# yflyzhang/RankPO

Hardware: AMD Instinct MI355X
Metric: query-passage pairs/sec (higher is better)
Workload: dtype bf16

## Files before the change

include/rankpo_hip.h:

```cpp
#ifndef RANKPO_HIP_H
#define RANKPO_HIP_H

#include <stddef.h>
#include <stdint.h>

#ifdef __cplusplus
extern "C" {
#endif

typedef void* rpo_stream_t;

typedef enum {
    RPO_OK = 0,
    RPO_ERR_INVALID_ARG = -1,
    RPO_ERR_UNSUPPORTED = -2,
    RPO_ERR_WORKSPACE = -3,
    RPO_ERR_LAUNCH = -4
} rpo_status;

typedef enum { RPO_DT_F32 = 0, RPO_DT_BF16 = 1, RPO_DT_F16 = 2 } rpo_dtype;
typedef enum { RPO_POOL_LAST = 0, RPO_POOL_CLS = 1 } rpo_pool_mode;
typedef enum { RPO_TARGET_INBATCH = 0, RPO_TARGET_FIRST = 1 } rpo_target_mode;
typedef enum { RPO_LOSS_SIGMOID = 0, RPO_LOSS_HINGE = 1 } rpo_loss_type;

// ... 86 lines not shown
                          int dtype, float lr, float beta1, float beta2, float eps, float weight_decay, const void* ls_state,
                          rpo_stream_t stream);

int rpo_swiglu_fwd(const void* g, const void* u, void* out, int64_t rows, int64_t cols, int64_t ld_gu, int64_t ld_out,
                   int dtype, rpo_stream_t stream);
int rpo_swiglu_bwd(const void* g, const void* u, const void* dout, void* dg, void* du, void* prod_out, int64_t rows,
                   int64_t cols, int64_t ld_gu, int64_t ld_dout, int64_t ld_dgu, int64_t ld_prod, int dtype,
                   rpo_stream_t stream);
int rpo_swiglu_bwd_t(const void* g, const void* u, const void* dout, void* dg, void* du, void* prod_t_out, void* dgu_t_out,
                     int64_t rows, int64_t cols, int64_t ld_gu, int64_t ld_dout, int64_t ld_dgu, int64_t ld_t, int dtype,
                     rpo_stream_t stream);
int rpo_rope(const void* x_in, void* x_out, int64_t row_stride, const float* cos_tab, const float* sin_tab,
             int64_t rows, int64_t heads, int64_t head_dim, int64_t period, int dtype, int backward,
             rpo_stream_t stream);

int rpo_transpose(const void* in, void* out, int64_t rows, int64_t cols, int64_t ld_in, int64_t ld_out, int dtype,
                  rpo_stream_t stream);

int rpo_add_rmsnorm_waves(int64_t rows);
int rpo_add_rmsnorm_fwd(const void* x, const void* delta, const void* weight, float eps, void* x_out, void* y_out,
                        float* rstd_out, int64_t rows, int64_t d, int dtype, rpo_stream_t stream);
int rpo_add_rmsnorm_bwd(const void* dy, const void* x_new, const void* weight, const float* rstd, const void* dres,
                        void* dx_out, float* dw_partial, int64_t rows, int64_t d, int dtype, rpo_stream_t stream);

int rpo_flash_attn_fwd(const void* q, const void* k, const void* v, int64_t q_stride, int64_t k_stride,
                       int64_t v_stride, const int* cu_seqlens, const int* tiles, int64_t ntiles, int64_t tile_cols,
                       int64_t total_tokens,
                       int64_t num_heads, int64_t num_kv_heads, int64_t head_dim, float scale, void* out,
                       int64_t out_stride, float* lse, int64_t lse_max_len, const float* rope_cos, const float* rope_sin,
                       int64_t rope_period, int64_t q_block, rpo_stream_t stream);

int rpo_flash_attn_bwd(const void* q, const void* k, const void* v, const void* out, const void* dout, int64_t q_stride,
                       int64_t k_stride, int64_t v_stride, int64_t out_stride, int64_t dout_stride,
                       const int* cu_seqlens, const int* q_tiles, int64_t n_q_tiles, int64_t q_tile_cols, const int* k_tiles,
                       int64_t n_k_tiles, int64_t key_block, int64_t sweep_down, int64_t total_tokens, int64_t num_heads,
                       int64_t num_kv_heads, int64_t head_dim, float scale, const float* lse, float* delta, void* dq, void* dk, void* dv,
                       int64_t dq_stride, int64_t dk_stride, int64_t dv_stride, const float* rope_cos, const float* rope_sin,
                       int64_t rope_period, int64_t q_block, rpo_stream_t stream);

int rpo_lastq_attn_fwd(const void* q, int64_t q_stride, const void* k, const void* v, int64_t k_stride, int64_t v_stride,
                       const int* cu_seqlens, int64_t num_seqs, int64_t num_heads, int64_t num_kv_heads, int64_t head_dim,
                       float scale, void* out, int64_t out_stride, float* lse, rpo_stream_t stream);
int rpo_lastq_attn_bwd(const void* q, int64_t q_stride, const void* k, const void* v, int64_t k_stride, int64_t v_stride,
                       const int* cu_seqlens, int64_t num_seqs, int64_t num_heads, int64_t num_kv_heads, int64_t head_dim,
                       float scale, const void* out, int64_t out_stride, const void* dout, int64_t dout_stride, const float* lse,
                       void* dq, int64_t dq_stride, void* dk, void* dv, int64_t dk_stride, int64_t dv_stride, rpo_stream_t stream);
// ... 65 lines not shown
                 int dtype, rpo_stream_t stream);

float rpo_hidden_dropout_scale(float p_drop);
int rpo_add_layernorm_drop_fwd(const void* a, int64_t lda, const void* b, int64_t ldb, const void* gamma, const void* beta,
                               float eps, void* y, int64_t ldy, void* s, int64_t lds, int64_t rows, int64_t d, int dtype,
                               float p_drop, uint64_t seed, int64_t site, rpo_stream_t stream);
int rpo_bert_embed_ln_drop_fwd(const int* ids, const int* token_types, const int* pos, int64_t tokens, const void* word,
                               int64_t vocab, const void* type_emb, int64_t n_types, const void* pos_emb, int64_t n_pos,
                               const void* gamma, const void* beta, float eps, void* y, int64_t ldy, void* s, int64_t lds,
                               int64_t d, int dtype, float p_drop, uint64_t seed, int64_t site, rpo_stream_t stream);
int rpo_layernorm_drop_bwd(const void* s, int64_t lds, const void* gamma, const void* dy, int64_t lddy, float eps, void* ds,
                           int64_t ldds, void* db, int64_t lddb, float* dgamma_partial, float* dbeta_partial, int64_t rows,
                           int64_t d, int dtype, float p_drop, uint64_t seed, int64_t site_in, int64_t site_out,
                           rpo_stream_t stream);
int rpo_hidden_dropout_mask(int64_t row0, int64_t rows, int64_t d, float p_drop, uint64_t seed, int64_t site,
                            unsigned char* mask, rpo_stream_t stream);

int64_t rpo_embed_grad_workspace_elems(int64_t n_partials, int64_t d);
int rpo_embed_grad_sorted(const void* ds, int64_t ldds, int64_t tokens, int64_t d, int dtype, const int* order, const int* chunks,
                          int64_t n_chunks, const int* multi, int64_t n_multi, int64_t n_partials, void* out, int64_t ldout,
                          int64_t table_rows, int64_t padding_idx, float* workspace, int64_t workspace_elems,
                          rpo_stream_t stream);

int rpo_topk_merge(const void* scores, int64_t ld, int64_t rows, int64_t cols, int64_t col0, int k, int dtype,
                   float* best_val, int64_t* best_idx, int first, rpo_stream_t stream);
int rpo_topk_merge_split(const void* scores, int64_t ld, int64_t rows, int64_t cols, int64_t col0, int k, int dtype, int split,
                         float* best_val, int64_t* best_idx, int first, rpo_stream_t stream);

int rpo_sim_topk_filter_ok(int64_t Q, int64_t P, int64_t d);
int rpo_sim_topk_filter(const void* q, const void* p, int64_t Q, int64_t P, int64_t d, int dtype, int64_t col0, int k,
                        int round_scores, const float* best_val, const int64_t* best_idx, float* cand_val, int64_t* cand_idx,
                        int32_t* cand_cnt, int cap, rpo_stream_t stream);
int rpo_sim_scores_f32(const void* q, const void* p, int64_t Q, int64_t P, int64_t d, int dtype, float* scores, int64_t ldc,
                       rpo_stream_t stream);
int rpo_topk_merge_candidates(const float* cand_val, const int64_t* cand_idx, int32_t* cand_cnt, int64_t rows, int cap, int k,
                              float* best_val, int64_t* best_idx, int32_t* overflow, rpo_stream_t stream);

int rpo_split_bf16x3(const float* x, int64_t ldx, int64_t rows, int64_t d, void* planes, int64_t ldp, int32_t* inexact,
                     rpo_stream_t stream);
int rpo_sim_planes_ok(int64_t Q, int64_t P, int64_t d);
int rpo_sim_scores_f32_planes(const void* q, const void* p, int64_t Q, int64_t P, int64_t d, float* scores, int64_t ldc,
                              rpo_stream_t stream);
int rpo_sim_topk_filter_planes(const void* q, const void* p, int64_t Q, int64_t P, int64_t d, int64_t col0, int k,
                               const float* best_val, const int64_t* best_idx, float* cand_val, int64_t* cand_idx,
                               int32_t* cand_cnt, int cap, rpo_stream_t stream);

// ... 5 lines not shown
```

rankpo_amd/_lib.py:

```python
from __future__ import annotations

import ctypes as C
import os

_HERE = os.path.dirname(os.path.abspath(__file__))
LIB_PATH = os.path.join(_HERE, "csrc", "librankpo_hip.so")

RPO_OK = 0
RPO_DT_F32, RPO_DT_BF16, RPO_DT_F16 = 0, 1, 2
RPO_POOL_LAST, RPO_POOL_CLS = 0, 1
(RPO_LS_SCALE, RPO_LS_MULT, RPO_LS_NORM, RPO_LS_SKIP, RPO_LS_GOOD_STEPS, RPO_LS_CUR_HYSTERESIS, RPO_LS_APPLIED_STEPS,
 RPO_LS_SKIPPED_STEPS, RPO_LS_FLOOR_HITS) = range(9)
RPO_LS_WORDS = 16
RPO_TARGET_INBATCH, RPO_TARGET_FIRST = 0, 1
RPO_LOSS_SIGMOID, RPO_LOSS_HINGE = 0, 1
RPO_BUILD_ONEWAVE64 = 1
RPO_NUM_METRICS = 9
METRIC_KEYS = (
    "rankpo_loss", "sft_loss", "rewards/chosen", "rewards/rejected", "rewards/accuracies",
    "rewards/margins", "scores/chosen", "scores/rejected", "scores/margins",
)


class RankPOParams(C.Structure):
# ... 75 lines not shown
                                           _i32, _f32, _f32, _u64, _vp, _i64, _vp, _vp]),
    "rpo_bidir_attn_bwd": (C.c_int, [_vp, _vp, _vp, _i64, _i64, _i64, _vp, _i64, _vp, _i64, _vp, _vp, _vp, _vp, _i64, _vp, _i64,
                                     _i64, _i64, _i64, _i64, _i64, _i64, _i32, _f32, _f32, _u64, _vp, _i64, _vp, _i64, _vp, _i64,
                                     _vp]),
    "rpo_bidir_attn_dropout_mask": (C.c_int, [_i64, _i64, _i64, _i64, _i64, _i64, _f32, _u64, _vp, _vp]),
    "rpo_add_layernorm_train_fwd": (C.c_int, [_vp, _i64, _vp, _i64, _vp, _vp, _f32, _vp, _i64, _vp, _i64, _i64, _i64, _i32, _vp]),
    "rpo_bert_embed_ln_train_fwd": (C.c_int, [_vp, _vp, _vp, _i64, _vp, _i64, _vp, _i64, _vp, _i64, _vp, _vp, _f32, _vp, _i64, _vp,
                                              _i64, _i64, _i32, _vp]),
    "rpo_layernorm_bwd_blocks": (C.c_int, [_i64]),
    "rpo_layernorm_bwd": (C.c_int, [_vp, _i64, _vp, _vp, _i64, _f32, _vp, _i64, _vp, _vp, _i64, _i64, _i32, _vp]),
    "rpo_gelu_out_fwd": (C.c_int, [_vp, _i64, _vp, _i64, _i64, _i64, _i32, _vp]),
    "rpo_gelu_bwd": (C.c_int, [_vp, _i64, _vp, _i64, _vp, _i64, _i64, _i64, _i32, _vp]),
    "rpo_hidden_dropout_scale": (_f32, [_f32]),
    "rpo_add_layernorm_drop_fwd": (C.c_int, [_vp, _i64, _vp, _i64, _vp, _vp, _f32, _vp, _i64, _vp, _i64, _i64, _i64, _i32, _f32, _u64,
                                             _i64, _vp]),
    "rpo_bert_embed_ln_drop_fwd": (C.c_int, [_vp, _vp, _vp, _i64, _vp, _i64, _vp, _i64, _vp, _i64, _vp, _vp, _f32, _vp, _i64, _vp,
                                             _i64, _i64, _i32, _f32, _u64, _i64, _vp]),
    "rpo_layernorm_drop_bwd": (C.c_int, [_vp, _i64, _vp, _vp, _i64, _f32, _vp, _i64, _vp, _i64, _vp, _vp, _i64, _i64, _i32, _f32,
                                         _u64, _i64, _i64, _vp]),
    "rpo_hidden_dropout_mask": (C.c_int, [_i64, _i64, _i64, _f32, _u64, _i64, _vp, _vp]),
    "rpo_embed_grad_workspace_elems": (_i64, [_i64, _i64]),
    "rpo_embed_grad_sorted": (C.c_int, [_vp, _i64, _i64, _i64, _i32, _vp, _vp, _i64, _vp, _i64, _i64, _vp, _i64, _i64, _i64, _vp,
                                        _i64, _vp]),
}

_lib = None


def load():
    global _lib
    if _lib is not None:
        return _lib
    if not os.path.exists(LIB_PATH):
        raise ImportError(
            f"{LIB_PATH} not found: the HIP scoring library is not built.  Run "
            "`python -c 'import __graft_entry__ as g; g.build()'` (or `make -C rankpo_amd/csrc`).  "
            "rankpo_amd has no CPU fallback for its hot path.")
    import torch
    lib = C.CDLL(LIB_PATH)
    for name, (res, args) in SIGNATURES.items():
        try:
            fn = getattr(lib, name)
        except AttributeError as e:
            raise ImportError(f"{LIB_PATH} does not export {name}; rebuild it (make -C rankpo_amd/csrc)") from e
        fn.restype = res
        fn.argtypes = args
# ... 11 lines not shown
```

rankpo_amd/csrc/embed_grad.hip:

```cpp
#include "common.hpp"

namespace {

constexpr int kEgWaves = 4;
constexpr int kEgSliceCols = 512;

template <typename T> __device__ __forceinline__ void add_row(float (&acc)[8], const Vec16<T>& x) {
#pragma unroll
    for (int j = 0; j < 8; ++j) acc[j] += x.v[j];
}

template <typename T> __device__ __forceinline__ void store_rounded(T* p, const float (&acc)[8]) {
    Vec16<T> r;
#pragma unroll
    for (int j = 0; j < 8; ++j) r.v[j] = acc[j];
    r.store(p);
}

template <typename T>
__global__ __launch_bounds__(64 * kEgWaves) void embed_grad_chunk_kernel(
    const T* __restrict__ ds, int64_t ldds, int tokens, int d, const int* __restrict__ order, const int* __restrict__ chunks,
    int64_t n_chunks, int64_t n_partials, T* __restrict__ out, int64_t ldout, int64_t table_rows, int64_t padding_idx,
    float* __restrict__ ws) {
    const int wave = __builtin_amdgcn_readfirstlane((int)(threadIdx.x >> 6));
// ... 45 lines not shown
    const int* __restrict__ multi, int64_t n_multi, int d, int64_t n_partials, const float* __restrict__ ws,
    T* __restrict__ out, int64_t ldout, int64_t table_rows, int64_t padding_idx) {
    const int wave = __builtin_amdgcn_readfirstlane((int)(threadIdx.x >> 6));
    const int64_t m = (int64_t)blockIdx.x * kEgWaves + wave;
    if (m >= n_multi) return;
    const int slice = (int)blockIdx.y;
    const int* mu = multi + 3 * m;
    const int row = mu[0], slot0 = mu[1], k = mu[2];
    if (row < 0 || row >= table_rows || row == padding_idx || slot0 < 0 || k < 1 || (int64_t)slot0 + k > n_partials) return;
    const int col = slice * kEgSliceCols + (int)(threadIdx.x & 63) * 8;
    if (col >= d) return;
    const float* p = ws + (int64_t)slot0 * d + col;
    float acc[8];
#pragma unroll
    for (int j = 0; j < 8; ++j) acc[j] = 0.f;
    for (int i = 0; i < k; ++i, p += d) {
        const float4 a = *reinterpret_cast<const float4*>(p), b = *reinterpret_cast<const float4*>(p + 4);
        acc[0] += a.x; acc[1] += a.y; acc[2] += a.z; acc[3] += a.w;
        acc[4] += b.x; acc[5] += b.y; acc[6] += b.z; acc[7] += b.w;
    }
    store_rounded<T>(out + (int64_t)row * ldout + col, acc);
}

}

extern "C" int64_t rpo_embed_grad_workspace_elems(int64_t n_partials, int64_t d) {
    return n_partials <= 0 || d <= 0 ? 0 : n_partials * d;
}

extern "C" int rpo_embed_grad_sorted(const void* ds, int64_t ldds, int64_t tokens, int64_t d, int dtype, const int* order,
                                     const int* chunks, int64_t n_chunks, const int* multi, int64_t n_multi, int64_t n_partials,
                                     void* out, int64_t ldout, int64_t table_rows, int64_t padding_idx, float* workspace,
                                     int64_t workspace_elems, rpo_stream_t stream) {
    if (!ds || !out || tokens < 0 || tokens > INT32_MAX || d <= 0 || table_rows <= 0 || table_rows > INT32_MAX || ldds < d ||
        ldout < d || !rpo_dtype_ok(dtype) || n_chunks < 0 || n_multi < 0 || n_partials < 0 || padding_idx < -1 ||
        padding_idx >= table_rows || (n_chunks > 0 && (!order || !chunks)) || (n_multi > 0 && !multi) ||
        (n_partials > 0 && !workspace) || (n_multi > 0) != (n_partials > 0))
        return RPO_ERR_INVALID_ARG;
    if (dtype == RPO_DT_F32 || d % 8 || d > 65535 * (int64_t)kEgSliceCols) return RPO_ERR_UNSUPPORTED;
    if (!rpo_aligned16(ds) || !rpo_aligned16(out) || ldds % 8 || ldout % 8 || (n_partials > 0 && !rpo_aligned16(workspace)))
        return RPO_ERR_UNSUPPORTED;
    if (workspace_elems < rpo_embed_grad_workspace_elems(n_partials, d)) return RPO_ERR_WORKSPACE;
    if (tokens == 0 || n_chunks == 0) return RPO_OK;
    const unsigned nslices = (unsigned)rpo_cdiv(d, kEgSliceCols);
    if (n_chunks > INT32_MAX || n_multi > INT32_MAX) return RPO_ERR_UNSUPPORTED;
    const dim3 block(64 * kEgWaves), grid1((unsigned)rpo_cdiv(n_chunks, kEgWaves), nslices),
// ... 19 lines not shown
```

rankpo_amd/csrc/encoder_ops.hip:

```cpp
#include "common.hpp"

namespace {

constexpr int kEwThreads = 256;

__device__ __forceinline__ float sigmoid_f(float x) { return 1.0f / (1.0f + __expf(-x)); }

template <typename T>
__global__ __launch_bounds__(kEwThreads) void swiglu_fwd_kernel(const T* __restrict__ g, const T* __restrict__ u,
                                                                T* __restrict__ out, int64_t rows, int vec_per_row,
                                                                int64_t ld_gu, int64_t ld_out) {
    constexpr int V = Elem<T>::kVec;
    const int64_t i = (int64_t)blockIdx.x * kEwThreads + threadIdx.x;
    const int64_t r = i / vec_per_row;
    if (r >= rows) return;
    const int c = (int)(i - r * vec_per_row) * V;
    Vec16<T> a, b, o;
    a.load_nt(g + r * ld_gu + c);
    b.load_nt(u + r * ld_gu + c);
#pragma unroll
    for (int k = 0; k < V; ++k) o.v[k] = a.v[k] * sigmoid_f(a.v[k]) * b.v[k];
    o.store_nt(out + r * ld_out + c);
}

// ... 551 lines not shown
        (delta && (!rpo_aligned16(delta) || !rpo_aligned16(x_out))))
        return RPO_ERR_UNSUPPORTED;
    hipStream_t st = (hipStream_t)stream;
    const int nw = norm_waves(rows, RPO_NORM_FWD_CAP);
    if (dtype == RPO_DT_BF16) return launch_norm_fwd<bf16_t>(x, delta, weight, eps, x_out, y_out, rstd_out, rows, d, nw, st);
    if (dtype == RPO_DT_F32) return launch_norm_fwd<float>(x, delta, weight, eps, x_out, y_out, rstd_out, rows, d, nw, st);
    return RPO_ERR_INVALID_ARG;
}

extern "C" int rpo_add_rmsnorm_bwd(const void* dy, const void* x_new, const void* weight, const float* rstd,
                                   const void* dres, void* dx_out, float* dw_partial, int64_t rows, int64_t d,
                                   int dtype, rpo_stream_t stream) {
    if (!dy || !x_new || !weight || !rstd || !dx_out || !dw_partial || rows <= 0 || d <= 0) return RPO_ERR_INVALID_ARG;
    const int V = dtype == RPO_DT_BF16 ? 8 : 4;
    if (d % V != 0 || !rpo_aligned16(dy) || !rpo_aligned16(x_new) || !rpo_aligned16(dx_out) || !rpo_aligned16(weight) ||
        !rpo_aligned16(dw_partial) || (dres && !rpo_aligned16(dres)))
        return RPO_ERR_UNSUPPORTED;
    hipStream_t st = (hipStream_t)stream;
    const int nw = rpo_add_rmsnorm_waves(rows);
    if (dtype == RPO_DT_BF16) return launch_norm_bwd<bf16_t>(dy, x_new, weight, rstd, dres, dx_out, dw_partial, rows, d, nw, st);
    if (dtype == RPO_DT_F32) return launch_norm_bwd<float>(dy, x_new, weight, rstd, dres, dx_out, dw_partial, rows, d, nw, st);
    return RPO_ERR_INVALID_ARG;
}
```

rankpo_amd/encoder.py:

```python
from __future__ import annotations

import functools
import json
import math
import os
from types import SimpleNamespace
from typing import Optional

import torch
import torch.nn.functional as F
from torch import nn
from torch.utils.checkpoint import checkpoint

from . import ops as _ops


class EncoderConfig(SimpleNamespace):

    def to_dict(self):
        return dict(self.__dict__)

    @classmethod
    def from_json_file(cls, path):
        with open(path) as f:
# ... 507 lines not shown
            o += n + 2
        if not all(oks):
            return None
        ids_parts, pos_parts = [], []
        for ids, m in batches:
            L = m.shape[1]
            flat = torch.nonzero(m.reshape(-1).to(torch.bool), as_tuple=False).squeeze(1)
            ids_parts.append(ids.reshape(-1)[flat])
            pos_parts.append(flat % L)
        n_fill = 0
        if (dev.type == "cuda" and self.embed_tokens.weight.dtype == torch.bfloat16 and sum(lens) >= 4096
                and self.pack_fill):
            n_fill = (-sum(lens)) % 256
        if n_fill:
            pad_id = self.config.pad_token_id if self.config.pad_token_id is not None else 0
            ids_parts.append(torch.full((n_fill,), pad_id, dtype=ids_parts[0].dtype, device=ids_parts[0].device))
            pos_parts.append(torch.arange(n_fill, dtype=pos_parts[0].dtype, device=pos_parts[0].device))
            lens = lens + [n_fill]
        ids = ids_parts[0] if len(ids_parts) == 1 else torch.cat(ids_parts)
        pos = pos_parts[0] if len(pos_parts) == 1 else torch.cat(pos_parts)
        if on_host:
            both = torch.stack([ids.to(torch.int32), pos.to(torch.int32)]).pin_memory().to(dev, non_blocking=True)
            ids, pos = both[0], both[1]
        x = self.embed_tokens(ids)[None]
        rope = self._rope(pos)
        N = len(lens)
        cu = torch.zeros(N + 1, dtype=torch.int32, device=x.device)
        cu[1:] = torch.tensor(lens, dtype=torch.int64).cumsum(0).to(torch.int32).to(x.device, non_blocking=True)
        tiles = k_tiles = fwd_tiles = None
        if (x.is_cuda and self.config.head_dim in (64, 128) and x.dtype == torch.bfloat16
                and self.hand_attention):
            tiles = _ops.attn_tile_table(lens, x.device, self.config.num_attention_heads, self.config.num_key_value_heads)
            if FWD128_ONE_WAVE:
                fwd_tiles = _ops.attn_fwd_tile_table(lens, x.device, self.config.num_attention_heads,
                                                     self.config.num_key_value_heads, self.config.head_dim)
            if torch.is_grad_enabled():
                k_tiles = _ops.attn_key_tile_table(
                    lens, x.device, self.config.num_key_value_heads,
                    _ops.ATTN_KEY_BLOCK if self.config.head_dim == 64 else _ops.ATTN_KEY_BLOCK_HD128)
        f32_tiles = f32_last_tiles = None
        if ((LLAMA_F32_ATTENTION or self.f32_attention) and x.is_cuda and x.dtype == torch.float32 and not torch.is_grad_enabled()
                and _ops.causal_attn_f32_shape_ok(self.config.num_attention_heads, self.config.num_key_value_heads,
                                                  self.config.head_dim)):
            f32_tiles = _ops.causal_attn_f32_tile_table(lens, lens, x.device)
            f32_last_tiles = _ops.causal_attn_f32_tile_table([1] * N, lens, x.device)
        f32_k_tiles = f32_last_k_tiles = None
        if ((LLAMA_F32_ATTENTION_TRAIN or self.f32_attention_train) and x.is_cuda and x.dtype == torch.float32
# ... 553 lines not shown
```

rankpo_amd/ops.py:

```python
from __future__ import annotations

import ctypes as C
import threading
from dataclasses import dataclass
from typing import NamedTuple

import torch

from . import _lib
from ._lib import (RPO_DT_BF16, RPO_DT_F16, RPO_DT_F32, RPO_LOSS_HINGE, RPO_LOSS_SIGMOID, RPO_NUM_METRICS, RPO_POOL_CLS,
                   RPO_POOL_LAST, RPO_TARGET_FIRST, RPO_TARGET_INBATCH, METRIC_KEYS, RankPOParams, check)

F_NORMALIZE_EPS = 1e-12


def _dt(t: torch.Tensor) -> int:
    if t.dtype == torch.float32:
        return RPO_DT_F32
    if t.dtype == torch.bfloat16:
        return RPO_DT_BF16
    if t.dtype == torch.float16:
        return RPO_DT_F16
    raise TypeError(f"rankpo_amd HIP kernels take float32, bfloat16 or float16 tensors, got {t.dtype}")


# ... 240 lines not shown


def rankpo_loss_metrics(q, p, cfg: RankPOConfig, ref_chosen=None, ref_rejected=None):
    return _RankPO.apply(q, p, ref_chosen, ref_rejected, cfg)


def _swiglu_fwd(lib, gu, prod, rows, ff):
    es = gu.element_size()
    with torch.cuda.device(gu.device):
        check(lib.rpo_swiglu_fwd(gu.data_ptr(), gu.data_ptr() + ff * es, prod.data_ptr(), rows, ff, 2 * ff, ff, _dt(gu),
                                 _stream(gu)), "rpo_swiglu_fwd")
    return prod


LINEAR_TN = True
WGRAD_MIXED = True
SWIGLU_DGU_T = True
SWIGLU_DGU_T_DEFAULT_MAX_BYTES = 6 * 2 ** 30
SWIGLU_DGU_T_MAX_BYTES = SWIGLU_DGU_T_DEFAULT_MAX_BYTES
SWIGLU_PROD_T = True
WGRAD_SPLIT_T = 4


def transpose2d(x):
    _need_gpu(x)
    lib = _lib.load()
    if x.dim() != 2 or x.stride(1) != 1:
        raise ValueError("transpose2d: a 2-D tensor with contiguous rows")
    R, C_ = x.shape
    out = torch.empty((C_, R), dtype=x.dtype, device=x.device)
    with torch.cuda.device(x.device):
        check(lib.rpo_transpose(x.data_ptr(), out.data_ptr(), R, C_, x.stride(0), R, _dt(x), _stream(x)), "rpo_transpose")
    return out


WGRAD_DY_T_HITS = 0


def wgrad(dy2, x2, dy_t=None):
    n, k = dy2.shape[1], x2.shape[1]
    if dy_t is not None and tuple(dy_t.shape) == (n, dy2.shape[0]) and dy_t.dtype == dy2.dtype and x2.stride(1) == 1:
        global WGRAD_DY_T_HITS
        WGRAD_DY_T_HITS += 1
        return torch.nn.functional.linear(dy_t, transpose2d(x2))
    if WGRAD_MIXED and dy2.is_cuda and dy2.dtype == torch.bfloat16 and dy2.stride(1) == 1 and x2.stride(1) == 1:
        if n >= 2 * k:
            return dy2.t() @ transpose2d(x2).t()
        if k >= 2 * n:
            return transpose2d(dy2) @ x2
        T, S = dy2.shape[0], WGRAD_SPLIT_T
        if S > 1 and T >= 32768 and T % S == 0 and n * k <= 8 * 1024 * 1024 and dy2.is_contiguous() and x2.is_contiguous():
            if _bmm_f32_out_ok(dy2.device):
                part = torch.bmm(dy2.view(S, T // S, n).transpose(1, 2), x2.view(S, T // S, k), out_dtype=torch.float32)
                return part.sum(0).to(dy2.dtype)
    return dy2.t() @ x2


_BMM_F32_OUT = {}


def _bmm_f32_out_ok(device) -> bool:
    key = str(device)
    if key not in _BMM_F32_OUT:
        try:
            a = torch.ones(2, 8, 16, dtype=torch.bfloat16, device=device)
            r = torch.bmm(a.transpose(1, 2), a, out_dtype=torch.float32)
            _BMM_F32_OUT[key] = bool(r.dtype == torch.float32 and float(r[0, 0, 0]) == 8.0)
        except Exception:
            _BMM_F32_OUT[key] = False
    return _BMM_F32_OUT[key]


def _wt(w):
    return transpose2d(w) if w.is_cuda and w.dtype in (torch.bfloat16, torch.float16, torch.float32) and w.stride(1) == 1 else w.t().contiguous()


# ... 132 lines not shown
        return x_new, y

    @staticmethod
    def backward(ctx, *grads):
        x_new, weight, rstd = ctx.saved_tensors
        lib = _lib.load()
        if ctx.has_delta:
            dres, dy = grads
        else:
            dres, dy = None, grads[0]
        d = x_new.shape[-1]
        rows = x_new.numel() // d
        if dy is None:
            return dres, (dres if ctx.has_delta else None), None, None
        dy = dy.contiguous()
        dres = None if dres is None else dres.contiguous()
        dx = torch.empty_like(x_new)
        nw = lib.rpo_add_rmsnorm_waves(rows)
        dwp = torch.empty((nw, d), dtype=torch.float32, device=x_new.device)
        with torch.cuda.device(x_new.device):
            check(lib.rpo_add_rmsnorm_bwd(dy.data_ptr(), x_new.data_ptr(), weight.data_ptr(), rstd.data_ptr(), _p(dres),
                                          dx.data_ptr(), dwp.data_ptr(), rows, d, _dt(x_new), _stream(x_new)),
                  "rpo_add_rmsnorm_bwd")
        dw = dwp.sum(0).to(weight.dtype) if ctx.needs_input_grad[2] else None
        return dx, (dx if ctx.has_delta else None), dw, None


def add_rmsnorm(x, delta, weight, eps):
    if delta is None:
        return x, _AddRMSNorm.apply(x, None, weight, eps)
    return _AddRMSNorm.apply(x, delta, weight, eps)


def fused_norm_ok(x) -> bool:
    if not x.is_cuda or x.dtype not in (torch.float32, torch.bfloat16):
        return False
    v = 8 if x.dtype == torch.bfloat16 else 4
    d = x.shape[-1]
    return d % v == 0 and d // v <= 64 * 8


class _Rope(torch.autograd.Function):

    @staticmethod
    def forward(ctx, x, cos, sin, heads, head_dim, grad_inplace):
        lib = _lib.load()
        row_len = x.shape[-1]
# ... 876 lines not shown
    return _AddLayerNorm.apply(a, b, weight, bias, eps, p_drop, seed, site)


def embed_grad_sorted(ds, plan: EmbedGradPlan, table_rows: int, padding_idx=None):
    lib = _lib.load()
    T, d = ds.shape
    if plan.order.shape[0] != T:
        raise ValueError("embed_grad_sorted: the plan was built for another number of tokens")
    ds = ds if ds.stride(1) == 1 and ds.stride(0) % 8 == 0 and ds.data_ptr() % 16 == 0 else ds.contiguous()
    out = torch.zeros((table_rows, d), dtype=ds.dtype, device=ds.device)
    if T == 0:
        return out
    ws_elems = lib.rpo_embed_grad_workspace_elems(plan.n_partials, d)
    ws = torch.empty((ws_elems,), dtype=torch.float32, device=ds.device) if ws_elems else None
    with torch.cuda.device(ds.device):
        check(lib.rpo_embed_grad_sorted(ds.data_ptr(), ds.stride(0), T, d, _dt(ds), plan.order.data_ptr(), plan.chunks.data_ptr(),
                                        plan.chunks.shape[0], plan.multi.data_ptr() if plan.multi.shape[0] else None,
                                        plan.multi.shape[0], plan.n_partials, out.data_ptr(), d, table_rows,
                                        -1 if padding_idx is None else int(padding_idx), _p(ws), ws_elems, _stream(ds)),
              "rpo_embed_grad_sorted")
    return out


class _BertEmbedLayerNorm(torch.autograd.Function):

    @staticmethod
    def forward(ctx, ids, pos, token_types, word, type_emb, pos_emb, weight, bias, eps, padding_idx, p_drop=0.0, seed=0,
                plans=None):
        lib = _lib.load()
        T, d = ids.shape[0], word.shape[1]
        for t in (word, type_emb, pos_emb):
            if not t.is_contiguous():
                raise ValueError("bert_embed_ln_train: embedding tables must be contiguous")
        y = torch.empty((T, d), dtype=word.dtype, device=word.device)
        s = torch.empty((T, d), dtype=word.dtype, device=word.device)
        ctx.drop = (float(p_drop), int(seed), bert_hidden_site()) if p_drop > 0 else None
        with torch.cuda.device(word.device):
            if ctx.drop is None:
                check(lib.rpo_bert_embed_ln_train_fwd(ids.data_ptr(), _p(token_types), pos.data_ptr(), T, word.data_ptr(),
                                                      word.shape[0], type_emb.data_ptr(), type_emb.shape[0], pos_emb.data_ptr(),
                                                      pos_emb.shape[0], weight.data_ptr(), bias.data_ptr(), float(eps),
                                                      y.data_ptr(), d, s.data_ptr(), d, d, _dt(word), _stream(word)),
                      "rpo_bert_embed_ln_train_fwd")
            else:
                check(lib.rpo_bert_embed_ln_drop_fwd(ids.data_ptr(), _p(token_types), pos.data_ptr(), T, word.data_ptr(),
                                                     word.shape[0], type_emb.data_ptr(), type_emb.shape[0], pos_emb.data_ptr(),
# ... 276 lines not shown
```

Before: 55.28.

## Add device-side sorted-run embedding gradient and native slab-sum reduction kernel

```diff
diff --git a/include/rankpo_hip.h b/include/rankpo_hip.h
--- a/include/rankpo_hip.h
+++ b/include/rankpo_hip.h
@@ -132,6 +132,11 @@
                         float* rstd_out, int64_t rows, int64_t d, int dtype, rpo_stream_t stream);
 int rpo_add_rmsnorm_bwd(const void* dy, const void* x_new, const void* weight, const float* rstd, const void* dres,
                         void* dx_out, float* dw_partial, int64_t rows, int64_t d, int dtype, rpo_stream_t stream);
+
+int64_t rpo_sum_slabs_group(int64_t S);
+size_t rpo_sum_slabs_workspace_bytes(int64_t S, int64_t n);
+int rpo_sum_slabs(const float* partials, void* out, int64_t S, int64_t n, int out_dtype, void* workspace,
+                  size_t workspace_bytes, rpo_stream_t stream);
 
 int rpo_flash_attn_fwd(const void* q, const void* k, const void* v, int64_t q_stride, int64_t k_stride,
                        int64_t v_stride, const int* cu_seqlens, const int* tiles, int64_t ntiles, int64_t tile_cols,
@@ -243,6 +248,11 @@
                           int64_t table_rows, int64_t padding_idx, float* workspace, int64_t workspace_elems,
                           rpo_stream_t stream);
 
+int64_t rpo_embed_grad_runs_workspace_elems(int64_t tokens, int64_t d);
+int rpo_embed_grad_runs(const void* ds, int64_t ldds, int64_t tokens, int64_t d, int dtype, const void* sorted_ids, int id_bytes,
+                        const int64_t* order, void* out, int64_t ldout, int64_t table_rows, int64_t padding_idx,
+                        float* workspace, int64_t workspace_elems, rpo_stream_t stream);
+
 int rpo_topk_merge(const void* scores, int64_t ld, int64_t rows, int64_t cols, int64_t col0, int k, int dtype,
                    float* best_val, int64_t* best_idx, int first, rpo_stream_t stream);
 int rpo_topk_merge_split(const void* scores, int64_t ld, int64_t rows, int64_t cols, int64_t col0, int k, int dtype, int split,
diff --git a/rankpo_amd/_lib.py b/rankpo_amd/_lib.py
--- a/rankpo_amd/_lib.py
+++ b/rankpo_amd/_lib.py
@@ -121,6 +121,11 @@
     "rpo_embed_grad_workspace_elems": (_i64, [_i64, _i64]),
     "rpo_embed_grad_sorted": (C.c_int, [_vp, _i64, _i64, _i64, _i32, _vp, _vp, _i64, _vp, _i64, _i64, _vp, _i64, _i64, _i64, _vp,
                                         _i64, _vp]),
+    "rpo_embed_grad_runs_workspace_elems": (_i64, [_i64, _i64]),
+    "rpo_embed_grad_runs": (C.c_int, [_vp, _i64, _i64, _i64, _i32, _vp, _i32, _vp, _vp, _i64, _i64, _i64, _vp, _i64, _vp]),
+    "rpo_sum_slabs_group": (_i64, [_i64]),
+    "rpo_sum_slabs_workspace_bytes": (_sz, [_i64, _i64]),
+    "rpo_sum_slabs": (C.c_int, [_vp, _vp, _i64, _i64, _i32, _vp, _sz, _vp]),
 }
 
 _lib = None
diff --git a/rankpo_amd/csrc/embed_grad.hip b/rankpo_amd/csrc/embed_grad.hip
--- a/rankpo_amd/csrc/embed_grad.hip
+++ b/rankpo_amd/csrc/embed_grad.hip
@@ -91,6 +91,167 @@
     store_rounded<T>(out + (int64_t)row * ldout + col, acc);
 }
 
+constexpr int kEgRunChunk = 32;
+
+template <bool I64> __device__ __forceinline__ int64_t eg_id(const void* ids, int64_t p) {
+    if constexpr (I64) return static_cast<const int64_t*>(ids)[p];
+    else return static_cast<const int*>(ids)[p];
+}
+
+template <typename T> __device__ __forceinline__ void eg_add(float (&acc)[8], const Vec16<T>& x) {
+#pragma unroll
+    for (int j = 0; j < Elem<T>::kVec; ++j) acc[j] += x.v[j];
+}
+
+template <typename T>
+__device__ __forceinline__ void eg_add_rows(float (&acc)[8], const T* __restrict__ src, int64_t ldds, int tokens,
+                                            const int64_t* __restrict__ order, int64_t p0, int64_t p1) {
+    int64_t p = p0;
+    for (; p + 4 <= p1; p += 4) {
+        Vec16<T> x[4];
+#pragma unroll
+        for (int u = 0; u < 4; ++u) {
+            int64_t t = order[p + u];
+            t = t < 0 ? 0 : (t >= tokens ? tokens - 1 : t);
+            x[u].load(src + t * ldds);
+        }
+#pragma unroll
+        for (int u = 0; u < 4; ++u) eg_add<T>(acc, x[u]);
+    }
+    for (; p < p1; ++p) {
+        int64_t t = order[p];
+        t = t < 0 ? 0 : (t >= tokens ? tokens - 1 : t);
+        Vec16<T> x;
+        x.load(src + t * ldds);
+        eg_add<T>(acc, x);
+    }
+}
+
+template <typename T> __device__ __forceinline__ void eg_store_rounded(T* p, const float (&acc)[8]) {
+    Vec16<T> r;
+#pragma unroll
+    for (int j = 0; j < Elem<T>::kVec; ++j) r.v[j] = acc[j];
+    r.store(p);
+}
+template <int V> __device__ __forceinline__ void eg_store_f32(float* p, const float (&acc)[8]) {
+#pragma unroll
+    for (int h = 0; h < V / 4; ++h)
+        *reinterpret_cast<float4*>(p + 4 * h) = make_float4(acc[4 * h], acc[4 * h + 1], acc[4 * h + 2], acc[4 * h + 3]);
+}
+
+template <typename T, bool I64>
+__global__ __launch_bounds__(64 * kEgWaves) void embed_grad_runs_kernel(
+    const T* __restrict__ ds, int64_t ldds, int tokens, int d, const void* __restrict__ ids, const int64_t* __restrict__ order,
+    T* __restrict__ out, int64_t ldout, int64_t table_rows, int64_t padding_idx, float* __restrict__ ws) {
+    constexpr int V = Elem<T>::kVec;
+    const int wave = __builtin_amdgcn_readfirstlane((int)(threadIdx.x >> 6));
+    const int64_t c = (int64_t)blockIdx.x * kEgWaves + wave;
+    const int64_t p0 = c * kEgRunChunk;
+    if (p0 >= tokens) return;
+    const int64_t p1 = p0 + kEgRunChunk < tokens ? p0 + kEgRunChunk : tokens;
+    const int col = (int)blockIdx.y * (64 * V) + (int)(threadIdx.x & 63) * V;
+    if (col >= d) return;
+    const bool head_open = p0 > 0 && eg_id<I64>(ids, p0 - 1) == eg_id<I64>(ids, p0);
+    const bool tail_open = p1 < tokens && eg_id<I64>(ids, p1) == eg_id<I64>(ids, p1 - 1);
+    float* wsc = ws + c * 2 * (int64_t)d + col;
+    for (int64_t p = p0; p < p1;) {
+        const int64_t id = eg_id<I64>(ids, p);
+        int64_t e = p + 1;
+        while (e < p1 && eg_id<I64>(ids, e) == id) ++e;
+        float acc[8];
+#pragma unroll
+        for (int j = 0; j < 8; ++j) acc[j] = 0.f;
+        eg_add_rows<T>(acc, ds + col, ldds, tokens, order, p, e);
+        if (p == p0 && head_open) eg_store_f32<V>(wsc, acc);
+        else if (e == p1 && tail_open) eg_store_f32<V>(wsc + d, acc);
+        else if (id >= 0 && id < table_rows && id != padding_idx) eg_store_rounded<T>(out + id * ldout + col, acc);
+        p = e;
+    }
+}
+
+template <typename T, bool I64>
+__global__ __launch_bounds__(64 * kEgWaves) void embed_grad_runs_join_kernel(
+    int tokens, int d, const void* __restrict__ ids, const float* __restrict__ ws, T* __restrict__ out, int64_t ldout,
+    int64_t table_rows, int64_t padding_idx) {
+    constexpr int V = Elem<T>::kVec;
+    const int wave = __builtin_amdgcn_readfirstlane((int)(threadIdx.x >> 6));
+    const int64_t c = (int64_t)blockIdx.x * kEgWaves + wave;
+    const int64_t p0 = c * kEgRunChunk, p1 = p0 + kEgRunChunk;
+    if (p1 >= tokens) return;
+    const int64_t id = eg_id<I64>(ids, p1 - 1);
+    if (eg_id<I64>(ids, p1) != id) return;
+    if (eg_id<I64>(ids, p0) == id && p0 > 0 && eg_id<I64>(ids, p0 - 1) == id) return;
+    if (id < 0 || id >= table_rows || id == padding_idx) return;
+    const int col = (int)blockIdx.y * (64 * V) + (int)(threadIdx.x & 63) * V;
+    if (col >= d) return;
+    int64_t k = 1;
+    while ((c + k + 1) * kEgRunChunk < tokens && eg_id<I64>(ids, (c + k + 1) * kEgRunChunk) == id) ++k;
+    float acc[8];
+#pragma unroll
+    for (int j = 0; j < 8; ++j) acc[j] = 0.f;
+    Vec16<float> x;
+#pragma unroll
+    for (int h = 0; h < V / 4; ++h) {
+        x.load(ws + (c * 2 + 1) * (int64_t)d + col + 4 * h);
+#pragma unroll
+        for (int j = 0; j < 4; ++j) acc[4 * h + j] += x.v[j];
+    }
+    for (int64_t i = 1; i <= k; ++i) {
+        const float* p = ws + (c + i) * 2 * (int64_t)d + col;
+#pragma unroll
+        for (int h = 0; h < V / 4; ++h) {
+            x.load(p + 4 * h);
+#pragma unroll
+            for (int j = 0; j < 4; ++j) acc[4 * h + j] += x.v[j];
+        }
+    }
+    eg_store_rounded<T>(out + id * ldout + col, acc);
+}
+
+}
+
+extern "C" int64_t rpo_embed_grad_runs_workspace_elems(int64_t tokens, int64_t d) {
+    return tokens <= 0 || d <= 0 ? 0 : rpo_cdiv(tokens, kEgRunChunk) * 2 * d;
+}
+
+extern "C" int rpo_embed_grad_runs(const void* ds, int64_t ldds, int64_t tokens, int64_t d, int dtype, const void* sorted_ids,
+                                   int id_bytes, const int64_t* order, void* out, int64_t ldout, int64_t table_rows,
+                                   int64_t padding_idx, float* workspace, int64_t workspace_elems, rpo_stream_t stream) {
+    if (!ds || !out || tokens < 0 || tokens > INT32_MAX || d <= 0 || table_rows <= 0 || table_rows > INT32_MAX || ldds < d ||
+        ldout < d || !rpo_dtype_ok(dtype) || padding_idx < -1 || padding_idx >= table_rows || (id_bytes != 4 && id_bytes != 8) ||
+        (tokens > 0 && (!sorted_ids || !order || !workspace)))
+        return RPO_ERR_INVALID_ARG;
+    const int V = dtype == RPO_DT_F32 ? 4 : 8;
+    if (d % 8 || d > 65535 * (int64_t)(64 * V)) return RPO_ERR_UNSUPPORTED;
+    if (!rpo_aligned16(ds) || !rpo_aligned16(out) || ldds % V || ldout % V || (tokens > 0 && !rpo_aligned16(workspace)))
+        return RPO_ERR_UNSUPPORTED;
+    if (workspace_elems < rpo_embed_grad_runs_workspace_elems(tokens, d)) return RPO_ERR_WORKSPACE;
+    if (tokens == 0) return RPO_OK;
+    const int64_t n_chunks = rpo_cdiv(tokens, kEgRunChunk);
+    const dim3 block(64 * kEgWaves), grid((unsigned)rpo_cdiv(n_chunks, kEgWaves), (unsigned)rpo_cdiv(d, 64 * V));
+    hipStream_t st = (hipStream_t)stream;
+#define RPO_EGR(T, I64)                                                                                                        \
+    do {                                                                                                                       \
+        RPO_LAUNCH((embed_grad_runs_kernel<T, I64>), grid, block, 0, st, (const T*)ds, ldds, (int)tokens, (int)d, sorted_ids,  \
+                   order, (T*)out, ldout, table_rows, padding_idx, workspace);                                                 \
+        if (n_chunks > 1) {                                                                                                    \
+            const int rc = rpo_launch_status();                                                                                \
+            if (rc != RPO_OK) return rc;                                                                                       \
+            RPO_LAUNCH((embed_grad_runs_join_kernel<T, I64>), grid, block, 0, st, (int)tokens, (int)d, sorted_ids,             \
+                       (const float*)workspace, (T*)out, ldout, table_rows, padding_idx);                                      \
+        }                                                                                                                      \
+    } while (0)
+#define RPO_EGR_T(T)                                                                                                           \
+    do {                                                                                                                       \
+        if (id_bytes == 8) RPO_EGR(T, true);                                                                                   \
+        else RPO_EGR(T, false);                                                                                                \
+    } while (0)
+    if (dtype == RPO_DT_F32) RPO_EGR_T(float);
+    else if (dtype == RPO_DT_BF16) RPO_EGR_T(bf16_t);
+    else RPO_EGR_T(f16_t);
+#undef RPO_EGR_T
+#undef RPO_EGR
+    return rpo_launch_status();
 }
 
 extern "C" int64_t rpo_embed_grad_workspace_elems(int64_t n_partials, int64_t d) {
diff --git a/rankpo_amd/csrc/encoder_ops.hip b/rankpo_amd/csrc/encoder_ops.hip
--- a/rankpo_amd/csrc/encoder_ops.hip
+++ b/rankpo_amd/csrc/encoder_ops.hip
@@ -597,3 +597,156 @@
     if (dtype == RPO_DT_F32) return launch_norm_bwd<float>(dy, x_new, weight, rstd, dres, dx_out, dw_partial, rows, d, nw, st);
     return RPO_ERR_INVALID_ARG;
 }
+
+namespace {
+
+constexpr int kSlabThreads = 256;
+constexpr int kSlabTileCols = 64;
+constexpr int kSlabFlatMax = 32;
+constexpr int kSlabMinGroup = 16;
+constexpr int kSlabMaxGroups = 64;
+
+template <typename T> __device__ __forceinline__ void store_rounded4(T* p, const float (&a)[4]) {
+    if constexpr (sizeof(T) == 4) {
+        *reinterpret_cast<float4*>(p) = make_float4(a[0], a[1], a[2], a[3]);
+    } else {
+        unsigned h[4];
+#pragma unroll
+        for (int j = 0; j < 4; ++j) {
+            T t;
+            Elem<T>::st(&t, a[j]);
+            h[j] = (unsigned)__builtin_bit_cast(unsigned short, t);
+        }
+        *reinterpret_cast<uint2*>(p) = make_uint2(h[0] | (h[1] << 16), h[2] | (h[3] << 16));
+    }
+}
+
+__device__ __forceinline__ void add_slabs(float (&acc)[4], const float* __restrict__ p, int64_t n, int s0, int s1) {
+    int s = s0;
+    for (; s + 8 <= s1; s += 8) {
+        Vec16<float> x[8];
+#pragma unroll
+        for (int u = 0; u < 8; ++u) x[u].load_nt(p + (int64_t)(s + u) * n);
+#pragma unroll
+        for (int u = 0; u < 8; ++u) {
+#pragma unroll
+            for (int j = 0; j < 4; ++j) acc[j] += x[u].v[j];
+        }
+    }
+    for (; s < s1; ++s) {
+        Vec16<float> x;
+        x.load_nt(p + (int64_t)s * n);
+#pragma unroll
+        for (int j = 0; j < 4; ++j) acc[j] += x.v[j];
+    }
+}
+
+template <typename T>
+__global__ __launch_bounds__(kSlabThreads) void sum_slabs_flat_kernel(const float* __restrict__ part, T* __restrict__ out, int S,
+                                                                      int64_t n) {
+    const int64_t col = ((int64_t)blockIdx.x * kSlabThreads + threadIdx.x) * 4;
+    if (col >= n) return;
+    float acc[4] = {0.f, 0.f, 0.f, 0.f};
+    add_slabs(acc, part + col, n, 0, S);
+    store_rounded4<T>(out + col, acc);
+}
+
+template <typename T>
+__global__ __launch_bounds__(64) void sum_slabs_tree_kernel(const float* __restrict__ part, T* __restrict__ out, int S, int64_t n,
+                                                            int group, float* gsum, unsigned* tickets) {
+    const int lane = (int)threadIdx.x;
+    const int64_t col = (int64_t)blockIdx.x * kSlabTileCols + lane;
+    const int g = (int)blockIdx.y, ngroups = (int)gridDim.y;
+    const bool own = col < n;
+    if (own) {
+        const int s0 = g * group, s1 = s0 + group < S ? s0 + group : S;
+        const float* p = part + col;
+        float acc = 0.f;
+        int s = s0;
+        for (; s + 16 <= s1; s += 16) {
+            float x[16];
+#pragma unroll
+            for (int u = 0; u < 16; ++u) x[u] = __builtin_nontemporal_load(p + (int64_t)(s + u) * n);
+#pragma unroll
+            for (int u = 0; u < 16; ++u) acc += x[u];
+        }
+        for (; s < s1; ++s) acc += __builtin_nontemporal_load(p + (int64_t)s * n);
+        __hip_atomic_store(reinterpret_cast<unsigned*>(gsum + (int64_t)g * n + col), __float_as_uint(acc), __ATOMIC_RELAXED,
+                           __HIP_MEMORY_SCOPE_AGENT);
+    }
+    asm volatile("s_waitcnt vmcnt(0)" ::: "memory");
+    int last = 0;
+    if (lane == 0)
+        last = __hip_atomic_fetch_add(tickets + blockIdx.x, 1u, __ATOMIC_RELAXED, __HIP_MEMORY_SCOPE_AGENT) + 1u == (unsigned)ngroups;
+    if (!__builtin_amdgcn_readfirstlane(last)) return;
+    __builtin_amdgcn_fence(__ATOMIC_ACQUIRE, "agent");
+    if (own) {
+        const unsigned* gp = reinterpret_cast<const unsigned*>(gsum) + col;
+        float acc = 0.f;
+        int k = 0;
+        for (; k + 16 <= ngroups; k += 16) {
+            float x[16];
+#pragma unroll
+            for (int u = 0; u < 16; ++u)
+                x[u] = __uint_as_float(__hip_atomic_load(gp + (int64_t)(k + u) * n, __ATOMIC_RELAXED, __HIP_MEMORY_SCOPE_AGENT));
+#pragma unroll
+            for (int u = 0; u < 16; ++u) acc += x[u];
+        }
+        for (; k < ngroups; ++k)
+            acc += __uint_as_float(__hip_atomic_load(gp + (int64_t)k * n, __ATOMIC_RELAXED, __HIP_MEMORY_SCOPE_AGENT));
+        Elem<T>::st(out + col, acc);
+    }
+}
+
+inline int64_t slab_group(int64_t S) {
+    if (S <= kSlabFlatMax) return S < 1 ? 1 : S;
+    const int64_t g = rpo_cdiv(S, kSlabMaxGroups);
+    return g < kSlabMinGroup ? kSlabMinGroup : g;
+}
+inline size_t slab_gsum_bytes(int64_t S, int64_t n) {
+    const int64_t g = slab_group(S);
+    return g >= S ? 0 : (size_t)((rpo_cdiv(S, g) * n * 4 + 15) / 16 * 16);
+}
+
+}
+
+extern "C" int64_t rpo_sum_slabs_group(int64_t S) { return slab_group(S); }
+
+extern "C" size_t rpo_sum_slabs_workspace_bytes(int64_t S, int64_t n) {
+    if (S < 1 || n < 1) return 0;
+    const size_t gs = slab_gsum_bytes(S, n);
+    return gs ? gs + (size_t)((rpo_cdiv(n, kSlabTileCols) * 4 + 15) / 16 * 16) : 0;
+}
+
+extern "C" int rpo_sum_slabs(const float* partials, void* out, int64_t S, int64_t n, int out_dtype, void* workspace,
+                             size_t workspace_bytes, rpo_stream_t stream) {
+    if (!partials || !out || S < 1 || n < 1 || !rpo_dtype_ok(out_dtype)) return RPO_ERR_INVALID_ARG;
+    if (n % 4 || S > (1 << 20) || !rpo_aligned16(partials) || !rpo_aligned16(out)) return RPO_ERR_UNSUPPORTED;
+    hipStream_t st = (hipStream_t)stream;
+    const int64_t group = slab_group(S);
+    if (group >= S) {
+        const int64_t nblk = rpo_cdiv(n / 4, kSlabThreads);
+        if (nblk > INT32_MAX) return RPO_ERR_UNSUPPORTED;
+        const dim3 grid((unsigned)nblk), block(kSlabThreads);
+        if (out_dtype == RPO_DT_F32) RPO_LAUNCH(sum_slabs_flat_kernel<float>, grid, block, 0, st, partials, (float*)out, (int)S, n);
+        else if (out_dtype == RPO_DT_BF16) RPO_LAUNCH(sum_slabs_flat_kernel<bf16_t>, grid, block, 0, st, partials, (bf16_t*)out, (int)S, n);
+        else RPO_LAUNCH(sum_slabs_flat_kernel<f16_t>, grid, block, 0, st, partials, (f16_t*)out, (int)S, n);
+        return rpo_launch_status();
+    }
+    const int64_t tiles = rpo_cdiv(n, kSlabTileCols), ngroups = rpo_cdiv(S, group);
+    if (tiles > INT32_MAX || ngroups > kSlabMaxGroups) return RPO_ERR_UNSUPPORTED;
+    if (!workspace || !rpo_aligned16(workspace)) return RPO_ERR_INVALID_ARG;
+    if (workspace_bytes < rpo_sum_slabs_workspace_bytes(S, n)) return RPO_ERR_WORKSPACE;
+    float* gsum = (float*)workspace;
+    unsigned* tickets = (unsigned*)((char*)workspace + slab_gsum_bytes(S, n));
+    (void)hipGetLastError();
+    if (hipMemsetAsync(tickets, 0, (size_t)((tiles * 4 + 15) / 16 * 16), st) != hipSuccess) return rpo_launch_status();
+    const dim3 grid((unsigned)tiles, (unsigned)ngroups), block(64);
+#define RPO_SS(T)                                                                                                              \
+    RPO_LAUNCH(sum_slabs_tree_kernel<T>, grid, block, 0, st, partials, (T*)out, (int)S, n, (int)group, gsum, tickets)
+    if (out_dtype == RPO_DT_F32) RPO_SS(float);
+    else if (out_dtype == RPO_DT_BF16) RPO_SS(bf16_t);
+    else RPO_SS(f16_t);
+#undef RPO_SS
+    return rpo_launch_status();
+}
diff --git a/rankpo_amd/encoder.py b/rankpo_amd/encoder.py
--- a/rankpo_amd/encoder.py
+++ b/rankpo_amd/encoder.py
@@ -553,7 +553,11 @@
         if on_host:
             both = torch.stack([ids.to(torch.int32), pos.to(torch.int32)]).pin_memory().to(dev, non_blocking=True)
             ids, pos = both[0], both[1]
-        x = self.embed_tokens(ids)[None]
+        if (_ops.EMBED_GRAD_DEVICE and torch.is_grad_enabled() and self.embed_tokens.weight.requires_grad
+                and _ops.embed_grad_device_takes(self.embed_tokens, ids)):
+            x = _ops.embedding_device_grad(self.embed_tokens, ids)[None]
+        else:
+            x = self.embed_tokens(ids)[None]
         rope = self._rope(pos)
         N = len(lens)
         cu = torch.zeros(N + 1, dtype=torch.int32, device=x.device)
diff --git a/rankpo_amd/ops.py b/rankpo_amd/ops.py
--- a/rankpo_amd/ops.py
+++ b/rankpo_amd/ops.py
@@ -1,6 +1,8 @@
 from __future__ import annotations
 
 import ctypes as C
+import functools
+import os
 import threading
 from dataclasses import dataclass
 from typing import NamedTuple
@@ -287,6 +289,41 @@
 WGRAD_SPLIT_T = 4
 
 
+def _env_switch(name: str, default: bool) -> bool:
+    v = os.environ.get("RPO_" + name)
+    return default if v is None else v.strip().lower() not in ("", "0", "false", "off", "no")
+
+
+SUM_SLABS_NATIVE = _env_switch("SUM_SLABS_NATIVE", False)
+EMBED_GRAD_DEVICE = _env_switch("EMBED_GRAD_DEVICE", True)
+
+
+def sum_slabs_ok(part) -> bool:
+    return (part.is_cuda and part.dtype == torch.float32 and part.dim() >= 2 and part.is_contiguous() and part.shape[0] >= 1
+            and part.shape[0] <= 1 << 20 and part[0].numel() >= 4 and part[0].numel() % 4 == 0)
+
+
+@functools.lru_cache(maxsize=256)
+def _sum_slabs_workspace_bytes(S: int, n: int) -> int:
+    return int(_lib.load().rpo_sum_slabs_workspace_bytes(S, n))
+
+
+def sum_slabs(part, dtype, workspace=None):
+    _need_gpu(part)
+    lib = _lib.load()
+    if part.dtype != torch.float32 or not part.is_contiguous() or part.dim() < 2:
+        raise ValueError("sum_slabs: a contiguous float32 tensor [S, ...]")
+    S, n = part.shape[0], part[0].numel()
+    out = torch.empty(part.shape[1:], dtype=dtype, device=part.device)
+    nbytes = _sum_slabs_workspace_bytes(S, n)
+    if nbytes and workspace is None:
+        workspace = torch.empty((nbytes,), dtype=torch.uint8, device=part.device)
+    with torch.cuda.device(part.device):
+        check(lib.rpo_sum_slabs(part.data_ptr(), out.data_ptr(), S, n, _dt(out), _p(workspace) if nbytes else None,
+                                workspace.numel() if nbytes else 0, _stream(part)), "rpo_sum_slabs")
+    return out
+
+
 def transpose2d(x):
     _need_gpu(x)
     lib = _lib.load()
@@ -317,6 +354,8 @@
         if S > 1 and T >= 32768 and T % S == 0 and n * k <= 8 * 1024 * 1024 and dy2.is_contiguous() and x2.is_contiguous():
             if _bmm_f32_out_ok(dy2.device):
                 part = torch.bmm(dy2.view(S, T // S, n).transpose(1, 2), x2.view(S, T // S, k), out_dtype=torch.float32)
+                if SUM_SLABS_NATIVE and sum_slabs_ok(part):
+                    return sum_slabs(part, dy2.dtype)
                 return part.sum(0).to(dy2.dtype)
     return dy2.t() @ x2
 
@@ -495,7 +534,12 @@
             check(lib.rpo_add_rmsnorm_bwd(dy.data_ptr(), x_new.data_ptr(), weight.data_ptr(), rstd.data_ptr(), _p(dres),
                                           dx.data_ptr(), dwp.data_ptr(), rows, d, _dt(x_new), _stream(x_new)),
                   "rpo_add_rmsnorm_bwd")
-        dw = dwp.sum(0).to(weight.dtype) if ctx.needs_input_grad[2] else None
+        if not ctx.needs_input_grad[2]:
+            dw = None
+        elif SUM_SLABS_NATIVE and sum_slabs_ok(dwp):
+            dw = sum_slabs(dwp, weight.dtype)
+        else:
+            dw = dwp.sum(0).to(weight.dtype)
         return dx, (dx if ctx.has_delta else None), dw, None
 
 
@@ -1418,6 +1462,60 @@
     return out
 
 
+@functools.lru_cache(maxsize=256)
+def _embed_grad_runs_workspace_elems(T: int, d: int) -> int:
+    return int(_lib.load().rpo_embed_grad_runs_workspace_elems(T, d))
+
+
+def embed_grad_device(ds, ids, table_rows: int, padding_idx=None):
+    _need_gpu(ds, ids)
+    lib = _lib.load()
+    T, d = ds.shape
+    if ids.dim() != 1 or ids.shape[0] != T or ids.dtype not in (torch.int32, torch.int64):
+        raise ValueError("embed_grad_device: ids must be an int32 / int64 vector with one entry per row of ds")
+    v = 4 if ds.dtype == torch.float32 else 8
+    ds = ds if ds.stride(1) == 1 and ds.stride(0) % v == 0 and ds.data_ptr() % 16 == 0 else ds.contiguous()
+    out = torch.zeros((table_rows, d), dtype=ds.dtype, device=ds.device)
+    if T == 0:
+        return out
+    sorted_ids, order = torch.sort(ids, stable=True)
+    ws_elems = _embed_grad_runs_workspace_elems(T, d)
+    ws = torch.empty((ws_elems,), dtype=torch.float32, device=ds.device)
+    with torch.cuda.device(ds.device):
+        check(lib.rpo_embed_grad_runs(ds.data_ptr(), ds.stride(0), T, d, _dt(ds), sorted_ids.data_ptr(), sorted_ids.element_size(),
+                                      order.data_ptr(), out.data_ptr(), d, table_rows,
+                                      -1 if padding_idx is None else int(padding_idx), ws.data_ptr(), ws_elems, _stream(ds)),
+              "rpo_embed_grad_runs")
+    return out
+
+
+def embed_grad_device_takes(emb, ids) -> bool:
+    w = emb.weight
+    return (w.is_cuda and ids.is_cuda and ids.dtype in (torch.int32, torch.int64) and ids.dim() == 1
+            and w.dtype in (torch.float32, torch.bfloat16, torch.float16) and w.dim() == 2 and w.shape[1] % 8 == 0
+            and w.is_contiguous() and not emb.sparse and emb.max_norm is None and not emb.scale_grad_by_freq)
+
+
+class _EmbeddingDeviceGrad(torch.autograd.Function):
+
+    @staticmethod
+    def forward(ctx, weight, ids, padding_idx):
+        ctx.save_for_backward(ids)
+        ctx.table_rows, ctx.padding_idx = weight.shape[0], padding_idx
+        return torch.nn.functional.embedding(ids, weight, padding_idx)
+
+    @staticmethod
+    def backward(ctx, dy):
+        ids, = ctx.saved_tensors
+        if not ctx.needs_input_grad[0]:
+            return None, None, None
+        return embed_grad_device(dy.reshape(-1, dy.shape[-1]), ids, ctx.table_rows, ctx.padding_idx), None, None
+
+
+def embedding_device_grad(emb, ids):
+    return _EmbeddingDeviceGrad.apply(emb.weight, ids, emb.padding_idx)
+
+
 class _BertEmbedLayerNorm(torch.autograd.Function):
 
     @staticmethod
```

Result: no change. 55.26 (-0.0%).
